# speechLabBcCuny/onssen

Measured on AMD Instinct MI355X. Metric: real_time_factor, higher is better.
Workload: dtype f32 as split-bf16 (bf16x3 MFMA, fp32 accumulate)

## Files before the change

### onssen_amd/_abi.py

```python
import ctypes as C
import os

EPI_BIAS, EPI_L2NORM, EPI_SIGMOID, EPI_RELU = 0, 1, 2, 3
EPI_BF16 = 0x100
ABI_VERSION = 14
WAV_TRUNCATED = 1
BLSTM_SPLIT_ROWS = 1
BLSTM_BF16X3 = 2
BLSTM_XCD = 4
BLSTM_FUSE_IN0 = 16
BLSTM_FUSE_TAIL = 32
BLSTM_BF16 = 64
BLSTM_G_READY = 128
BLSTM_WS_DIRTY = 65536
LSTM_BWD_STEPS, LSTM_BWD_XCD = 0, 1
DC_CLUSTER_LAUNCH_PER_ITERATION = 1
BLSTM_WS_HEADER = 32768
TASNET_GLN, TASNET_CLN, TASNET_BN = 0, 1, 2
TASNET_RELU, TASNET_SIGMOID, TASNET_SOFTMAX = 0, 1, 2
TASNET_RAGGED_MAX = 64
TASNET_F32, TASNET_BF16X3, TASNET_BF16 = 0, 1, 2

_vp, _i, _i64, _f, _sz = C.c_void_p, C.c_int, C.c_int64, C.c_float, C.c_size_t
_pp = C.POINTER(C.c_void_p)
# ... 508 lines not shown
    def cos_difference(self, s1, s2, n, out, stream):
        self.check(self.dll.onssen_cos_difference_f32(s1, s2, n, out, stream), "onssen_cos_difference_f32")

    def one_hot(self, feat, m1, m2, B, per_utt, db, utt_max, out, stream):
        self.check(self.dll.onssen_one_hot_f32(feat, m1, m2, B, per_utt, db, utt_max, out, stream), "onssen_one_hot_f32")

    def dc_compact_layout(self, B, T, F, D):
        co, do = _sz(), _sz()
        self.check(self.dll.onssen_dc_compact_layout(B, T, F, D, C.byref(co), C.byref(do)), "onssen_dc_compact_layout")
        return int(self.dll.onssen_dc_compact_workspace_bytes(B, T, F, D)), co.value, do.value

    def dc_index(self, feat, B, T, F, D, db, ws, ws_bytes, stream, frames=None):
        self.check(self.dll.onssen_dc_index_f32(feat, B, T, frames, F, D, db, ws, ws_bytes, stream), "onssen_dc_index_f32")

    def linear_x3p_compact(self, a_img, M, K, w_img, bias, N, group, eps, dest, dest_bs, F, comp, R, comp_bs, bf16_only, stream):
        self.check(self.dll.onssen_linear_x3p_compact(a_img, M, K, w_img, bias, N, group, eps, dest, dest_bs, F, comp, R, comp_bs,
                                                      int(bool(bf16_only)), stream), "onssen_linear_x3p_compact")

    def dc_cluster_compact(self, B, T, F, D, iters, masks, ws, ws_bytes, stream, flags=0, tol=1e-4):
        self.check(self.dll.onssen_dc_cluster_compact_f32(B, T, F, D, iters, tol, masks, ws, ws_bytes, flags, stream),
                   "onssen_dc_cluster_compact_f32")

    def dc_cluster(self, emb, feat, B, T, F, D, db, iters, masks, ws, ws_bytes, stream, flags=0, frames=None, tol=1e-4):
        if frames is not None:
            self.check(self.dll.onssen_dc_cluster_ragged_f32(emb, feat, B, T, frames, F, D, db, iters, tol, masks, ws, ws_bytes, flags,
                                                             stream), "onssen_dc_cluster_ragged_f32")
            return
        self.check(self.dll.onssen_dc_cluster_f32(emb, feat, B, T, F, D, db, iters, tol, masks, ws, ws_bytes, flags, stream),
                   "onssen_dc_cluster_f32")
```

### onssen_amd/csrc/gemm.inc

```
namespace lin {
constexpr int BM = 128, BN = 80, BK = 16;
constexpr int LD = 20;
constexpr int CLD = 84;
constexpr int STAGE = 2 * (BM + BN) * LD;
constexpr int SMEM = (BM * CLD > STAGE) ? BM * CLD : STAGE;
}

struct LinearArgs {
  const float* A;
  long a_s0, a_s1;
  const float* W;
  const float* bias;
  const float* resid;
  float* C;
  long c_s0, c_s1;
  int R, M, N, K, ldw, group;
  float eps;
};

__device__ __forceinline__ float f4c(const float4& v, int r) {
  return r == 0 ? v.x : (r == 1 ? v.y : (r == 2 ? v.z : v.w));
}

template <bool A_VEC, int MODE>
// ... 431 lines not shown
  long c_s0, c_s1;
  int R, M, N, KB, group;
  float eps;
  int tile_group;
  int c_vec;
  long a_bs, w_bs, c_bs;
  float* C2;
  long c2_s0, c2_s1, c2_bs;
  int n_split;
  int n_split_odd;
  const float* resid;
  int r_mod;
  const int* dest;
  long dest_bs;
  int F;
};

#ifndef ONSSEN_XP_ABLATE
#define ONSSEN_XP_ABLATE 0
#endif

template <int MODE, int WMS, int TERMS, bool BATCH = false>
__global__ __launch_bounds__(128 * WMS) void linear_x3p_kernel(LinearXpArgs p) {
  using namespace lxp;
  if constexpr (BATCH) {
    p.A += (long)blockIdx.z * p.a_bs;
    p.W += (long)blockIdx.z * p.w_bs;
    p.C += (long)blockIdx.z * p.c_bs;
    if (p.C2) p.C2 += (long)blockIdx.z * p.c2_bs;
    if (p.C2 && p.n_split_odd && (blockIdx.z & 1)) {
// ... 435 lines not shown
#define ONSSEN_XQ_STAGGER 0
#endif
#ifndef ONSSEN_XQ_WIDE_STORE
#define ONSSEN_XQ_WIDE_STORE 0
#endif
#ifndef ONSSEN_XQ_PRIO
#define ONSSEN_XQ_PRIO 0
#endif
#ifndef ONSSEN_XQ_STAGGER_PHASES
#define ONSSEN_XQ_STAGGER_PHASES 8
#endif
#define ONSSEN_EPI_L2NORM_SIGMOID 3
#define ONSSEN_EPI_L2NORM_COMPACT 4
namespace lxq {
constexpr int BM_MAX = 256;
}

template <int MODE, int TERMS, bool BATCH = false, int BN = 320, int BM = 256>
__global__ __launch_bounds__(512) void linear_x3q_kernel(LinearXpArgs p) {
  using namespace lxq;
  constexpr int STAGE = (BM + BN) * 128;
  constexpr int WN = BN / 4, NQW = (BM + BN) / 64;
  if constexpr (BATCH) {
    p.A += (long)blockIdx.z * p.a_bs;
    p.W += (long)blockIdx.z * p.w_bs;
    p.C += (long)blockIdx.z * p.c_bs;
  }
  constexpr int MT = BM / 32, NT = WN / 16, WM = BM / 2;
  __shared__ __attribute__((aligned(1024))) unsigned char stage0[STAGE];
  __shared__ __attribute__((aligned(1024))) unsigned char stage1[STAGE];
  const int tid = threadIdx.x, lane = tid & 63;
  const int wave = __builtin_amdgcn_readfirstlane(tid >> 6);
  const int wm = wave >> 2, wn = wave & 3;
  const int fi = lane & 15, fg = lane >> 4;
#if ONSSEN_XQ_STAGGER
  if (p.KB >= 16) {
    const int bl = blockIdx.y * gridDim.x + blockIdx.x;
    if (bl < 256) {
      const int ph = (bl >> 3) & (ONSSEN_XQ_STAGGER_PHASES - 1);
      for (int i = 0; i < ph; ++i) __builtin_amdgcn_s_sleep(ONSSEN_XQ_STAGGER);
    }
  }
#endif
  int n0, m0;
  {
    const int nbx = gridDim.x, nwg = nbx * gridDim.y, bid = blockIdx.y * nbx + blockIdx.x;
    const int q = nwg >> 3, r = nwg & 7, xcd = bid & 7;
    const int wg = (xcd < r ? xcd * (q + 1) : r * (q + 1) + (xcd - r) * q) + (bid >> 3);
    const int GN = p.tile_group, nby = gridDim.y;
    const int gfull = nbx / GN, nfull = gfull * GN * nby;
    int tn, tm;
    if (wg < nfull) {
      const int rem = wg % (nby * GN);
      tn = (wg / (nby * GN)) * GN + rem % GN;
      tm = rem / GN;
    } else {
      const int gl = nbx - gfull * GN, rem = wg - nfull;
      tn = gfull * GN + rem % gl;
      tm = rem / gl;
    }
    n0 = tn * BN;
    m0 = tm * BM;
  }
  const int pitch = p.KB * 128;
  const int a_rows = p.M - m0 < BM ? p.M - m0 : BM, w_rows = p.N - n0 < BN ? p.N - n0 : BN;
  const __amdgpu_buffer_rsrc_t ra = __builtin_amdgcn_make_buffer_rsrc(
      (void*)(p.A + (long)m0 * p.KB * 64), 0, a_rows * pitch, 0x00020000);
  const __amdgpu_buffer_rsrc_t rw = __builtin_amdgcn_make_buffer_rsrc(
      (void*)(p.W + (long)n0 * p.KB * 64), 0, w_rows * pitch, 0x00020000);
  const unsigned dma_lane = (unsigned)((lane >> 3) * pitch + (((lane & 7) ^ (lane >> 3)) * 16));
  auto dma = [&](unsigned char* stage, int kb) {
    const unsigned koff = (unsigned)(kb * 128);
#pragma unroll
    for (int j = 0; j < NQW; ++j) {
      const int q = wave * NQW + j;
      if (q < BM / 8)
        __builtin_amdgcn_raw_ptr_buffer_load_lds(ra, ONSSEN_LDS_PTR(stage + q * 1024), 16, dma_lane + (unsigned)(q * 8 * pitch) + koff, 0, 0, 0);
      else
        __builtin_amdgcn_raw_ptr_buffer_load_lds(rw, ONSSEN_LDS_PTR(stage + q * 1024), 16, dma_lane + (unsigned)((q - BM / 8) * 8 * pitch) + koff, 0, 0, 0);
    }
  };

  f32x4 acc[MT][NT];
#pragma unroll
  for (int mt = 0; mt < MT; ++mt)
#pragma unroll
    for (int nt = 0; nt < NT; ++nt) acc[mt][nt] = f32x4{0.f, 0.f, 0.f, 0.f};

  const unsigned ch = (unsigned)((fg ^ (fi & 7)) * 16), cl = ch ^ 64u;
  const unsigned fa_off = (unsigned)((wm * WM + fi) * 128);
  const unsigned fw_off = (unsigned)((BM + wn * WN + fi) * 128);
  auto compute = [&](const unsigned char* sb) {
    s16x8 wh[NT], wl[NT];
#pragma unroll
    for (int nt = 0; nt < NT; ++nt) {
// ... 40 lines not shown
      __builtin_amdgcn_s_waitcnt(0x0F70);
      __syncthreads();
    }
  }

  float4 bv[NT];
#pragma unroll
  for (int nt = 0; nt < NT; ++nt) {
    const int n = n0 + wn * WN + nt * 16 + 4 * fg;
    bv[nt].x = n + 0 < p.N ? p.bias[n + 0] : 0.f;
    bv[nt].y = n + 1 < p.N ? p.bias[n + 1] : 0.f;
    bv[nt].z = n + 2 < p.N ? p.bias[n + 2] : 0.f;
    bv[nt].w = n + 3 < p.N ? p.bias[n + 3] : 0.f;
  }
  u32x4 posv[MODE == ONSSEN_EPI_L2NORM_COMPACT ? MT : 1];
  if constexpr (MODE == ONSSEN_EPI_L2NORM_COMPACT) {
    const __amdgpu_buffer_rsrc_t rd = __builtin_amdgcn_make_buffer_rsrc((void*)p.dest, 0, (int)((long)p.R * p.dest_bs * 4 + 12), 0x00020000);
    const int f0 = (n0 + wn * WN) / p.group;
#pragma unroll
    for (int mt = 0; mt < MT; ++mt) {
      const int m = m0 + wm * WM + mt * 16 + fi;
      posv[mt] = __builtin_amdgcn_raw_buffer_load_b128(
          rd, m < p.M ? (unsigned)(((long)(m % p.R) * p.dest_bs + (long)(m / p.R) * p.F + f0) * 4) : 0x7ffffff0u, 0, 0);
    }
  }
#pragma unroll
  for (int mt = 0; mt < MT; ++mt) {
    const int m = m0 + wm * WM + mt * 16 + fi;
    float4 v[NT];
#pragma unroll
    for (int nt = 0; nt < NT; ++nt)
      v[nt] = make_float4(acc[mt][nt][0] + bv[nt].x, acc[mt][nt][1] + bv[nt].y, acc[mt][nt][2] + bv[nt].z,
                          acc[mt][nt][3] + bv[nt].w);
    if (MODE == ONSSEN_EPI_L2NORM && p.resid && m < p.M) {
      const float* rrow = p.resid + (long)(m / p.R) * p.c_s0 + (long)((m % p.R) % p.r_mod) * p.c_s1;
#pragma unroll
      for (int nt = 0; nt < NT; ++nt) {
        const int n = n0 + wn * WN + nt * 16 + 4 * fg;
// ... 38 lines not shown
        if (MODE == ONSSEN_EPI_L2NORM_SIGMOID && n0 + wn * WN + nt * 16 + 4 * fg >= p.n_split) {
          v[nt].x = 1.0f / (1.0f + expf(-v[nt].x)); v[nt].y = 1.0f / (1.0f + expf(-v[nt].y));
          v[nt].z = 1.0f / (1.0f + expf(-v[nt].z)); v[nt].w = 1.0f / (1.0f + expf(-v[nt].w));
        } else {
          v[nt].x *= sc; v[nt].y *= sc; v[nt].z *= sc; v[nt].w *= sc;
        }
      }
    } else if (MODE == ONSSEN_EPI_SIGMOID) {
#pragma unroll
      for (int nt = 0; nt < NT; ++nt) {
        v[nt].x = 1.0f / (1.0f + expf(-v[nt].x)); v[nt].y = 1.0f / (1.0f + expf(-v[nt].y));
        v[nt].z = 1.0f / (1.0f + expf(-v[nt].z)); v[nt].w = 1.0f / (1.0f + expf(-v[nt].w));
      }
    }
    if constexpr (MODE == ONSSEN_EPI_L2NORM_COMPACT) {
      if (m < p.M) {
        float* cb = p.C + (long)(m % p.R) * p.c_s1;
#pragma unroll
        for (int nt = 0; nt < NT; ++nt) {
          const int n = n0 + wn * WN + nt * 16 + 4 * fg, q = (nt * 16 + 4 * fg) / p.group;
          const int pos = (int)(q == 0 ? posv[mt][0] : q == 1 ? posv[mt][1] : q == 2 ? posv[mt][2] : posv[mt][3]);
          if (n < p.N && pos >= 0) *reinterpret_cast<float4*>(cb + (long)pos * p.group + (nt * 16 + 4 * fg) % p.group) = v[nt];
        }
      }
      continue;
    }
#if ONSSEN_XQ_WIDE_STORE
    if (MODE != ONSSEN_EPI_L2NORM_SIGMOID && p.c_vec) {
      const int mb = m0 + wm * WM + mt * 16, r8 = fi & 7;
      const int ma = mb + r8, mc = mb + r8 + 8;
      float* rowa = p.C + (long)(ma / p.R) * p.c_s0 + (long)(ma % p.R) * p.c_s1;
      float* rowc = p.C + (long)(mc / p.R) * p.c_s0 + (long)(mc % p.R) * p.c_s1;
// ... 292 lines not shown
```

### onssen_amd/csrc/labels_cluster.inc

```
__global__ void utt_max_kernel(const float* __restrict__ x, long per_utt, float* __restrict__ out) {
  __shared__ float red[256];
  const float* p = x + (long)blockIdx.x * per_utt;
  float m = -INFINITY;
  for (long i = threadIdx.x; i < per_utt; i += 256) m = fmaxf(m, p[i]);
  red[threadIdx.x] = m;
  __syncthreads();
  for (int s = 128; s > 0; s >>= 1) {
    if ((int)threadIdx.x < s) red[threadIdx.x] = fmaxf(red[threadIdx.x], red[threadIdx.x + s]);
    __syncthreads();
  }
  if (threadIdx.x == 0) out[blockIdx.x] = red[0];
}

__global__ void labels_kernel(const float* __restrict__ mix, const float* __restrict__ s1, const float* __restrict__ s2,
                              const float* __restrict__ feat, const float* __restrict__ fmax, long per_utt, long total,
                              float db_threshold, float* __restrict__ one_hot, float* __restrict__ mag_mix,
                              float* __restrict__ mag_s1, float* __restrict__ mag_s2, float* __restrict__ cos_s1,
                              float* __restrict__ cos_s2) {
  for (long e = (long)blockIdx.x * blockDim.x + threadIdx.x; e < total; e += (long)gridDim.x * blockDim.x) {
    const float xr = mix[2 * e], xi = mix[2 * e + 1];
    const float ar = s1[2 * e], ai = s1[2 * e + 1], br = s2[2 * e], bi = s2[2 * e + 1];
    const float m1 = hypotf(ar, ai), m2 = hypotf(br, bi);
    mag_mix[e] = hypotf(xr, xi);
    mag_s1[e] = m1;
// ... 727 lines not shown
  };
  if (fast) run(std::true_type{}); else run(std::false_type{});
  if (gave_up) return;
  if (j == 0) {
    if (tid < 2 * D) w[1 + tid] = cen[tid];
    if (tid == 0) {
      if (converged) w[ws_stride - 1] = 1.0f;
      iu[66] = it_done | (converged ? 0x10000 : 0) | (fast ? 0 : 0x20000);
    }
  }
}


__global__ __launch_bounds__(256) void kmeans2_index_kernel(const float* __restrict__ feat, long per_utt, float db,
                                                            const float* __restrict__ ws, long ws_stride, int* __restrict__ iw,
                                                            int* __restrict__ dest, const int* __restrict__ frames, int F, int D) {
  using namespace km;
  __shared__ int scan[256];
  __shared__ int base_s;
  const int b = blockIdx.y, tid = threadIdx.x;
  const float* f = feat + (long)b * per_utt;
  int* dst = dest + (long)b * per_utt;
  const float thr = ws[(long)b * ws_stride] - db / 20.0f;
  const long nb = frames ? (long)frames[b] * F : per_utt;
  const long chunk = (nb + NBLK - 1) / NBLK, i_lo = (long)blockIdx.x * chunk, i_hi = i_lo + chunk < nb ? i_lo + chunk : nb;
  if (tid == 0) {
    int sacc = 0;
    for (int k = 0; k < (int)blockIdx.x; ++k) sacc += iw[(long)b * IW + k];
    base_s = sacc;
    if (blockIdx.x == NBLK - 1) iw[(long)b * IW + 64] = sacc + iw[(long)b * IW + NBLK - 1];
  }
// ... 4 lines not shown
    const int act = (i < i_hi && f[i] >= thr) ? 1 : 0;
    scan[tid] = act;
    __syncthreads();
    for (int off = 1; off < 256; off <<= 1) {
      const int v = tid >= off ? scan[tid - off] : 0;
      __syncthreads();
      scan[tid] += v;
      __syncthreads();
    }
    if (i < i_hi) dst[i] = act ? base + scan[tid] - act : -1;
    const int tot = scan[255];
    __syncthreads();
    base += tot;
  }
  for (long i = nb + (long)blockIdx.x * 256 + tid; i < per_utt; i += (long)NBLK * 256) dst[i] = -1;
  if (blockIdx.x == 0) {
    float* wb = const_cast<float*>(ws) + (long)b * ws_stride;
    for (int k = tid; k < 2 * NBP * (D + 4); k += 256) wb[1 + 2 * D + k] = __builtin_bit_cast(float, 1u);
  }
}

template <int DT>
__global__ __launch_bounds__(256) void kmeans2_mask_compact_kernel(const float* __restrict__ comp, const int* __restrict__ dest,
                                                                   long per_utt, int D_rt, const float* __restrict__ ws,
                                                                   long ws_stride, float* __restrict__ masks) {
  using namespace km;
  constexpr int DC = DT ? DT : DMAX;
  const int D = DT ? DT : D_rt;
  const int b = blockIdx.y, tid = threadIdx.x;
  const float* e = comp + (long)b * per_utt * D;
  const int* dst = dest + (long)b * per_utt;
  const float* w = ws + (long)b * ws_stride;
  float c0[DC], c1[DC];
// ... 35 lines not shown
```

### onssen_amd/csrc/onssen_hip.hip

```cpp
#include <hip/hip_runtime.h>
#include <hip/hip_bf16.h>

#include <math.h>
#include <stdint.h>
#include <stdlib.h>

#include <type_traits>

#include "../../include/onssen_hip.h"

typedef float f32x4 __attribute__((vector_size(16)));
typedef unsigned int u32x4 __attribute__((vector_size(16)));
typedef unsigned int u32x2 __attribute__((vector_size(8)));
typedef short s16x8 __attribute__((vector_size(16)));
typedef __bf16 bf16x8_t __attribute__((vector_size(16)));

#ifdef ONSSEN_HOST_EMULATION
#define ONSSEN_USE_AFTER(x, after) ((void)0)
#define ONSSEN_LDS_PTR(p) ((void*)(p))
#else
#define ONSSEN_USE_AFTER(x, after) asm volatile("" : "+v"(x) : "v"(after))
#define ONSSEN_LDS_PTR(p) ((__attribute__((address_space(3))) void*)(p))
#endif

// ... 21 lines not shown
#define ONSSEN_LAUNCH_CHECK()                   \
  do {                                          \
    hipError_t e__ = hipGetLastError();         \
    if (e__ != hipSuccess) return (int)e__;     \
  } while (0)

static inline int ceil_div(int a, int b) { return (a + b - 1) / b; }
static inline size_t align256(size_t x) { return (x + 255) & ~(size_t)255; }
#ifdef ONSSEN_DEBUG_KNOBS
#define ONSSEN_KNOB_INT(name, dflt) (getenv(name) ? atoi(getenv(name)) : (dflt))
#else
#define ONSSEN_KNOB_INT(name, dflt) (dflt)
#endif
static inline bool aligned16(const void* p) { return (reinterpret_cast<uintptr_t>(p) & 15u) == 0; }
static inline bool aligned256(const void* p) { return (reinterpret_cast<uintptr_t>(p) & 255u) == 0; }
#ifndef ONSSEN_X3Q_SMALL_DEFAULT
#define ONSSEN_X3Q_SMALL_DEFAULT 0
#endif
#ifndef ONSSEN_X3R_DEFAULT
#define ONSSEN_X3R_DEFAULT 0
#endif

#include "pack.inc"
#include "gemm.inc"
#include "labels_cluster.inc"
#include "lstm.inc"
#include "lstm_bwd.inc"
#include "fft.inc"
#include "loss_sdr.inc"
#include "wav_io.inc"
// ... 351 lines not shown
                                   float* C2, int64_t c2_bs, int64_t c2_s0, int64_t c2_s1, int batch, void* stream,
                                   int n_split_odd = 0) {
  if (!a_img || !w_img || !bias || !C || M <= 0 || K <= 0 || N <= 0 || R <= 0 || batch <= 0 || batch > 65535) return ONSSEN_E_ARG;
  if (C2 && (n_split <= 0 || n_split >= N)) return ONSSEN_E_ARG;
  if (n_split_odd && (!C2 || n_split_odd < 0 || n_split_odd >= N)) return ONSSEN_E_ARG;
  if (!aligned16(a_img) || !aligned16(w_img) || (a_bs % 8) != 0 || (w_bs % 8) != 0) return ONSSEN_E_ALIGN;
  const int KB = ceil_div(K, 32);
  if ((long)lxp::BM * KB * 128 > 0x7fffffffL) return ONSSEN_E_ARG;
  ONSSEN_CLEAR_ERROR();
  LinearXpArgs p;
  p.A = a_img; p.W = w_img; p.bias = bias; p.C = C; p.c_s0 = (long)c_s0; p.c_s1 = (long)c_s1; p.R = R; p.M = M; p.N = N;
  p.KB = KB; p.group = 0; p.eps = 0.f; p.tile_group = 4;
  p.c_vec = !C2 && aligned16(C) && (N % 4) == 0 && (c_s0 % 4) == 0 && (c_s1 % 4) == 0 && (c_bs % 4) == 0;
  p.a_bs = (long)a_bs; p.w_bs = (long)w_bs; p.c_bs = (long)c_bs;
  p.C2 = C2; p.c2_s0 = (long)c2_s0; p.c2_s1 = (long)c2_s1; p.c2_bs = (long)c2_bs; p.n_split = n_split; p.n_split_odd = n_split_odd;
  p.resid = nullptr; p.r_mod = 1; p.dest = nullptr; p.dest_bs = 0; p.F = 0;
  const dim3 grid((unsigned)ceil_div(N, lxp::BN), (unsigned)ceil_div(M, lxp::BM), (unsigned)batch);
  hipLaunchKernelGGL((linear_x3p_kernel<ONSSEN_EPI_BIAS, 4, 3, true>), grid, dim3(512), 0, (hipStream_t)stream, p);
  ONSSEN_LAUNCH_CHECK();
  return ONSSEN_OK;
}

int onssen_linear_x3p_batched(const uint16_t* a_img, int64_t a_bs, int M, int K, const uint16_t* w_img, int64_t w_bs,
                              const float* bias, int N, float* C, int64_t c_bs, int64_t ldc, int batch, void* stream) {
  if (ldc < N) return ONSSEN_E_ARG;
  return linear_x3p_batched_impl(a_img, a_bs, M, K, w_img, w_bs, bias, N, 1, C, c_bs, ldc, 0, 0, nullptr, 0, 0, 0, batch, stream);
}

int onssen_linear_x3p_batched_split(const uint16_t* a_img, int64_t a_bs, int M, int K, const uint16_t* w_img, int64_t w_bs,
                                    const float* bias, int N, int R, float* C, int64_t c_bs, int64_t c_s0, int64_t c_s1,
                                    int n_split, float* C2, int64_t c2_bs, int64_t c2_s0, int64_t c2_s1, int batch, void* stream) {
// ... 71 lines not shown
  const bool bf16_only = (mode & ONSSEN_EPI_BF16) != 0;
  mode &= ~ONSSEN_EPI_BF16;
  const bool pairs = mode == ONSSEN_EPI_L2NORM && group == 2;
  if (mode == ONSSEN_EPI_L2NORM) {
    if (!pairs && (group <= 0 || (group % 4) != 0 || (80 % group) != 0 || 80 / group > 4)) return ONSSEN_E_ARG;
    if ((N % group) != 0) return ONSSEN_E_ARG;
  } else if (mode != ONSSEN_EPI_BIAS && mode != ONSSEN_EPI_SIGMOID) {
    return ONSSEN_E_ARG;
  }
  if (resid && (mode != ONSSEN_EPI_L2NORM || resid_mod <= 0)) return ONSSEN_E_ARG;
  if (inv_norm && (mode != ONSSEN_EPI_L2NORM || pairs)) return ONSSEN_E_ARG;
  ONSSEN_CLEAR_ERROR();
  LinearXpArgs p;
  p.A = a_img; p.W = w_img; p.bias = bias; p.C = C; p.c_s0 = (long)c_s0; p.c_s1 = (long)c_s1; p.R = R; p.M = M; p.N = N;
  p.KB = KB; p.group = group; p.eps = eps; p.resid = resid; p.r_mod = resid ? resid_mod : 1;
  p.dest = nullptr; p.dest_bs = 0; p.F = 0;
  p.a_bs = p.w_bs = p.c_bs = 0;
  p.C2 = inv_norm; p.c2_s0 = p.c2_s1 = p.c2_bs = 0; p.n_split = 0; p.n_split_odd = 0;
  static const int x3_gn = ONSSEN_KNOB_INT("ONSSEN_X3_GN", 4);
  p.tile_group = x3_gn < 1 ? 1 : x3_gn;
  p.c_vec = aligned16(C) && (N % 4) == 0 && (c_s0 % 4) == 0 && (c_s1 % 4) == 0;
  hipStream_t st = (hipStream_t)stream;
  const char* env_q = getenv("ONSSEN_X3Q");
  const char* env_bm = getenv("ONSSEN_X3Q_BM");
  const int use_q = (pairs || resid || inv_norm) ? 1 : env_q ? atoi(env_q) : 1, force_bm = env_bm ? atoi(env_bm) : 0;
  if ((pairs || resid || inv_norm) && (long)lxq::BM_MAX * KB * 128 > 0x7fffffffL) return ONSSEN_E_ARG;
  if (use_q && (long)lxq::BM_MAX * KB * 128 <= 0x7fffffffL) {
    int bm = 256, bn = 320;
    double best = 1e30;
    for (int cbm = 256; cbm >= 128; cbm -= 128)
      for (int cbn = 320; cbn >= 256; cbn -= 64) {
// ... 81 lines not shown
}

int onssen_linear_x3p_pair(const uint16_t* a_img, int M, int K, const uint16_t* w_img, const float* bias, int N, int n_split,
                           int group, float eps, float* C, int R, int64_t c_s0, int64_t c_s1, float* C2, int64_t c2_s0,
                           int64_t c2_s1, int bf16_only, void* stream) {
  if (!a_img || !w_img || !bias || !C || !C2 || R <= 0 || M <= 0 || K <= 0 || N <= 0) return ONSSEN_E_ARG;
  if (group <= 0 || (group % 4) != 0 || (80 % group) != 0 || 80 / group > 4) return ONSSEN_E_ARG;
  if (n_split <= 0 || n_split >= N || (n_split % group) != 0) return ONSSEN_E_ARG;
  if (!aligned16(a_img) || !aligned16(w_img)) return ONSSEN_E_ALIGN;
  const int KB = ceil_div(K, 32);
  if ((long)lxq::BM_MAX * KB * 128 > 0x7fffffffL) return ONSSEN_E_ARG;
  ONSSEN_CLEAR_ERROR();
  LinearXpArgs p;
  p.A = a_img; p.W = w_img; p.bias = bias; p.C = C; p.c_s0 = (long)c_s0; p.c_s1 = (long)c_s1; p.R = R; p.M = M; p.N = N;
  p.KB = KB; p.group = group; p.eps = eps; p.resid = nullptr; p.r_mod = 1;
  p.dest = nullptr; p.dest_bs = 0; p.F = 0;
  p.a_bs = p.w_bs = p.c_bs = 0;
  p.C2 = C2; p.c2_s0 = (long)c2_s0; p.c2_s1 = (long)c2_s1; p.c2_bs = 0; p.n_split = n_split; p.n_split_odd = 0;
  p.tile_group = 4;
  p.c_vec = aligned16(C) && (n_split % 4) == 0 && (c_s0 % 4) == 0 && (c_s1 % 4) == 0;
  const long t256 = (long)ceil_div(M, 256) * ceil_div(N, 320), t128 = (long)ceil_div(M, 128) * ceil_div(N, 320);
  const int bm = (double)ceil_div(t128, 256L) * 128 * 1.15 < (double)ceil_div(t256, 256L) * 256 ? 128 : 256;
  const dim3 gridq((unsigned)ceil_div(N, 320), (unsigned)ceil_div(M, bm));
  hipStream_t st = (hipStream_t)stream;
  if (bm == 256) { if (bf16_only) hipLaunchKernelGGL((linear_x3q_kernel<ONSSEN_EPI_L2NORM_SIGMOID, 1, false, 320, 256>), gridq, dim3(512), 0, st, p);
                   else hipLaunchKernelGGL((linear_x3q_kernel<ONSSEN_EPI_L2NORM_SIGMOID, 3, false, 320, 256>), gridq, dim3(512), 0, st, p); }
  else { if (bf16_only) hipLaunchKernelGGL((linear_x3q_kernel<ONSSEN_EPI_L2NORM_SIGMOID, 1, false, 320, 128>), gridq, dim3(512), 0, st, p);
         else hipLaunchKernelGGL((linear_x3q_kernel<ONSSEN_EPI_L2NORM_SIGMOID, 3, false, 320, 128>), gridq, dim3(512), 0, st, p); }
  ONSSEN_LAUNCH_CHECK();
  return ONSSEN_OK;
}
// ... 3 lines not shown
                              int bf16_only, void* stream) {
  if (!a_img || !w_img || !bias || !dest || !comp || R <= 0 || M <= 0 || K <= 0 || N <= 0 || F <= 0) return ONSSEN_E_ARG;
  if (group <= 0 || (group % 4) != 0 || (80 % group) != 0 || 80 / group > 4 || N != F * group) return ONSSEN_E_ARG;
  if (!aligned16(a_img) || !aligned16(w_img) || !aligned16(comp) || (comp_bs % 4) != 0) return ONSSEN_E_ALIGN;
  const int KB = ceil_div(K, 32);
  if ((long)lxq::BM_MAX * KB * 128 > 0x7fffffffL) return ONSSEN_E_ARG;
  ONSSEN_CLEAR_ERROR();
  LinearXpArgs p;
  p.A = a_img; p.W = w_img; p.bias = bias; p.C = comp; p.c_s0 = 0; p.c_s1 = (long)comp_bs; p.R = R; p.M = M; p.N = N;
  p.KB = KB; p.group = group; p.eps = eps; p.resid = nullptr; p.r_mod = 1;
  p.a_bs = p.w_bs = p.c_bs = 0;
  p.C2 = nullptr; p.c2_s0 = p.c2_s1 = p.c2_bs = 0; p.n_split = 0; p.n_split_odd = 0;
  p.dest = dest; p.dest_bs = (long)dest_bs; p.F = F;
  p.tile_group = 4;
  p.c_vec = 1;
  const long t256 = (long)ceil_div(M, 256) * ceil_div(N, 320), t128 = (long)ceil_div(M, 128) * ceil_div(N, 320);
  const int bm = (double)ceil_div(t128, 256L) * 128 * 1.15 < (double)ceil_div(t256, 256L) * 256 ? 128 : 256;
  const dim3 gridq((unsigned)ceil_div(N, 320), (unsigned)ceil_div(M, bm));
  hipStream_t st = (hipStream_t)stream;
  if (bm == 256) { if (bf16_only) hipLaunchKernelGGL((linear_x3q_kernel<ONSSEN_EPI_L2NORM_COMPACT, 1, false, 320, 256>), gridq, dim3(512), 0, st, p);
                   else hipLaunchKernelGGL((linear_x3q_kernel<ONSSEN_EPI_L2NORM_COMPACT, 3, false, 320, 256>), gridq, dim3(512), 0, st, p); }
  else { if (bf16_only) hipLaunchKernelGGL((linear_x3q_kernel<ONSSEN_EPI_L2NORM_COMPACT, 1, false, 320, 128>), gridq, dim3(512), 0, st, p);
         else hipLaunchKernelGGL((linear_x3q_kernel<ONSSEN_EPI_L2NORM_COMPACT, 3, false, 320, 128>), gridq, dim3(512), 0, st, p); }
  ONSSEN_LAUNCH_CHECK();
  return ONSSEN_OK;
}

int onssen_linear_x3p_resid(const uint16_t* a_img, int M, int K, const uint16_t* w_img, const float* bias, int N, int group,
                            float eps, const float* resid, int resid_mod, float* C, int R, int64_t c_s0, int64_t c_s1,
                            int bf16_only, void* stream) {
  if (group != 2 && (group <= 0 || (group % 4) != 0)) return ONSSEN_E_ARG;
  return linear_x3p_impl(a_img, M, K, w_img, bias, N, ONSSEN_EPI_L2NORM | (bf16_only ? ONSSEN_EPI_BF16 : 0), group, eps, resid,
// ... 950 lines not shown
    }
  } else {
    hipLaunchKernelGGL((kmeans2_search_kernel<1>), sgrid, dim3(256), 0, st, emb, feature, per_utt, D, db_threshold, w, stride, frames, F);
    hipLaunchKernelGGL((kmeans2_pick_kernel<1>), dim3((unsigned)B), dim3(64), 0, st, emb, per_utt, D, w, stride, (int*)nullptr);
    for (int it = 0; it < iters; ++it) {
      ONSSEN_KM_ASSIGN(0, (float*)nullptr);
      hipLaunchKernelGGL(kmeans2_update_kernel, dim3((unsigned)B), dim3(256), 0, st, D, km::NBLK, w, stride, tol);
    }
  }
  ONSSEN_KM_ASSIGN(1, masks);
#undef ONSSEN_KM_ASSIGN
  ONSSEN_LAUNCH_CHECK();
  return ONSSEN_OK;
}

size_t onssen_dc_compact_workspace_bytes(int B, int T, int F, int D) {
  const size_t base = onssen_dc_cluster_workspace_bytes(B, T, F, D);
  return base ? align256(base) + align256((size_t)B * T * F * sizeof(int32_t) + 16) : 0;
}

int onssen_dc_compact_layout(int B, int T, int F, int D, size_t* comp_offset, size_t* dest_offset) {
  if (onssen_dc_cluster_workspace_bytes(B, T, F, D) == 0) return ONSSEN_E_ARG;
  if (comp_offset) *comp_offset = align256(onssen_dc_cluster_status_offset(B, D) + 256);
  if (dest_offset) *dest_offset = align256(onssen_dc_cluster_workspace_bytes(B, T, F, D));
  return ONSSEN_OK;
}

int onssen_dc_index_f32(const float* feature, int B, int T, const int32_t* frames, int F, int D, float db_threshold, void* ws,
                        size_t ws_bytes, void* stream) {
  if (!feature || !ws || B <= 0 || T <= 0 || F <= 0 || D <= 0 || D > km::DMAX) return ONSSEN_E_ARG;
  if (ws_bytes < onssen_dc_compact_workspace_bytes(B, T, F, D)) return ONSSEN_E_WORKSPACE;
  if (reinterpret_cast<uintptr_t>(ws) & 255u) return ONSSEN_E_ALIGN;
  ONSSEN_CLEAR_ERROR();
  hipStream_t st = (hipStream_t)stream;
  const long per_utt = (long)T * F, stride = 1 + 2 * D + km::NBLK * 2 * (D + 1) + 1;
  float* w = (float*)ws;
  int* iw = (int*)((char*)ws + align256(dc_cluster_header_floats(B, D) * sizeof(float)));
  size_t dest_off = 0;
  onssen_dc_compact_layout(B, T, F, D, nullptr, &dest_off);
  int* dest = (int*)((char*)ws + dest_off);
  const dim3 sgrid(km::NBLK, (unsigned)B);
  hipLaunchKernelGGL((kmeans2_search_kernel<0>), sgrid, dim3(256), 0, st, (const float*)nullptr, feature, per_utt, D, db_threshold, w, stride, frames, F);
  hipLaunchKernelGGL((kmeans2_count_kernel<true>), sgrid, dim3(256), 0, st, feature, per_utt, db_threshold, w, stride, iw, frames, F, D);
  hipLaunchKernelGGL(kmeans2_index_kernel, sgrid, dim3(256), 0, st, feature, per_utt, db_threshold, (const float*)w, stride, iw, dest, frames, F, D);
  ONSSEN_LAUNCH_CHECK();
  return ONSSEN_OK;
}

int onssen_dc_cluster_compact_f32(int B, int T, int F, int D, int iters, float tol, float* masks, void* ws, size_t ws_bytes,
                                  int flags, void* stream) {
  if (!masks || !ws || B <= 0 || T <= 0 || F <= 0 || D <= 0 || D > km::DMAX || iters < 0 || !(tol >= 0.f)) return ONSSEN_E_ARG;
  if (flags & ONSSEN_DC_CLUSTER_LAUNCH_PER_ITERATION) return ONSSEN_E_ARG;
  if (ws_bytes < onssen_dc_compact_workspace_bytes(B, T, F, D)) return ONSSEN_E_WORKSPACE;
  if (reinterpret_cast<uintptr_t>(ws) & 255u) return ONSSEN_E_ALIGN;
  ONSSEN_CLEAR_ERROR();
  hipStream_t st = (hipStream_t)stream;
  const long per_utt = (long)T * F, stride = 1 + 2 * D + km::NBLK * 2 * (D + 1) + 1;
  float* w = (float*)ws;
  int* iw = (int*)((char*)ws + align256(dc_cluster_header_floats(B, D) * sizeof(float)));
// ... 104 lines not shown
```

### onssen_amd/options.py

```python
import os

_BOOL = {True: "1", False: "0", "1": "1", "0": "0", "true": "1", "false": "0", "on": "1", "off": "0"}


def _choice(*allowed):
    def conv(v):
        v = str(v).lower() if not isinstance(v, bool) else _BOOL[v]
        if v not in allowed:
            raise ValueError(f"must be one of {allowed}, got {v!r}")
        return v
    return conv


def _flag(v):
    try:
        return _BOOL[v if isinstance(v, bool) else str(v).lower()]
    except KeyError:
        raise ValueError(f"must be a boolean, got {v!r}") from None


def _alias(table):
    def conv(v):
        k = _BOOL.get(v, None) if isinstance(v, bool) else str(v).lower()
        if k in table:
# ... 23 lines not shown
    "split_rows": ("ONSSEN_SPLIT_ROWS", "0", _flag, "launch-per-step recurrence: split the batch rows over two workgroups"),
    "ablate": ("ONSSEN_ABLATE", "0", _int, "profiling-only ablation bits of the recurrence kernels"),
    "serialize_persistent": ("ONSSEN_XCD_SERIALIZE", "0", _flag, "one persistent launch in flight per device across streams"),
    "nonfinite": ("ONSSEN_NONFINITE", "propagate", _choice("raise", "propagate"),
                  "non-finite activations seen by a persistent launch (they cannot pass its tagged exchange): propagate (default since round 6) = the "
                  "call is re-run on the launch-per-step recurrence, which gives nn.LSTM's NaN in / NaN out -- the reference's behaviour --; "
                  "raise = stop with an error instead"),
    "check": ("ONSSEN_CHECK", "0", _flag, "synchronise and examine the persistent launches' status words after every forward"),
    "check_weights": ("ONSSEN_CHECK_WEIGHTS", "0", _flag, "verify the packed weight images against the parameters before every forward (one synchronisation each: debugging)"),
    "weight_guard": ("ONSSEN_WEIGHT_GUARD", "1", _flag, "every inference forward that reuses cached weight images compares a device-side sampled checksum of the "
                     "live parameters with the one taken when the images were built (one small launch, no synchronisation); a mismatch drops the "
                     "images and raises StalePackedWeights at the next status poll (separate_* / tester.eval re-run the call by themselves)"),
    "dc_cluster": ("ONSSEN_DC_PERSISTENT", "1", _alias({"persistent": "1", "steps": "0"}),
                   "deep-clustering 2-means: all Lloyd passes in one launch, or one launch per pass"),
    "dc_compact": ("ONSSEN_DC_COMPACT", "1", _flag, "fc_dc stores only the active bins' embeddings into the clustering's array"),
    "train_blstm": ("ONSSEN_TRAIN_HIP", "1", _alias({"hip": "1", "aten": "0"}), "training BLSTM / head / BatchNorm on the HIP kernels"),
    "train_backward": ("ONSSEN_BWD_XCD", "1", _alias({"persistent": "1", "steps": "0"}), "backward recurrence form"),
    "train_gemm": ("ONSSEN_TRAIN_GEMM", "x3", _choice("x3", "blas"), "weight / input gradient contractions: package GEMM or library fp32"),
    "train_dp_image": ("ONSSEN_TRAIN_DP_IMAGE", "1", _flag, "the backward recurrence writes dP as the gradient GEMMs' x3 image instead of fp32"),
    "train_wgrad_rows": ("ONSSEN_TRAIN_WGRAD_ROWS", "1", _flag, "weight gradients from the row-major images the forward left"),
    "train_fused_loss": ("ONSSEN_TRAIN_FUSED_LOSS", "1", _flag, "fc_dc + normalise + loss_dc as one autograd node in train_step"),
    "train_fused_norm": ("ONSSEN_TRAIN_FUSED_NORM", "1", _flag, "fc_dc + normalise as one autograd node"),
    "tasnet_train": ("ONSSEN_TASNET_TRAIN", "hip", _choice("hip", "aten"),
                     "ConvTasNet training: hip = forward and backward of the network on the HIP kernels behind one autograd node "
                     "(gln / cln; bn, an input that requires a gradient and anomaly mode go to ATen by themselves), aten = autograd over PyTorch ops"),
    "loss": ("ONSSEN_LOSS_HIP", "1", _alias({"hip": "1", "torch": "0"}), "loss kernels on the device or PyTorch ops"),
    "fused_adam": ("ONSSEN_FUSED_ADAM", "1", _flag, "build_optimizer returns utils.ClipAdam (clipping + Adam on onssen_clip_adam_f32) for device parameters"),
    "cpu_autograd": ("ONSSEN_CPU_AUTOGRAD", "0", _flag, "TEST SCAFFOLDING, off in the product: let a training forward on CPU tensors run on ATen's LSTM so that "
                     "the multi-process logic (gradient buckets, replica agreement) can be exercised over gloo without a GPU; otherwise a CPU tensor raises"),
    "synthetic_data": ("ONSSEN_SYNTHETIC_DATA", "0", _flag, "wsj0_2mix_dataloader falls back to the synthetic corpus when data_path is empty"),
# ... 3 lines not shown
}

_configured = {}


def get(key):
    env, default, _, _ = TABLE[key]
    v = os.environ.get(env)
    if v is not None:
        return v
    return _configured.get(key, default)


def flag(key):
    return get(key) == "1"


def configure(**kw):
    old = {}
    for k, v in kw.items():
        if k not in TABLE:
            raise KeyError(f"onssen_amd.options: unknown option {k!r} (known: {sorted(TABLE)})")
        old[k] = _configured.get(k)
        if v is None:
            _configured.pop(k, None)
            continue
        try:
            _configured[k] = TABLE[k][2](v)
        except ValueError as e:
            raise ValueError(f"onssen_amd.options: {k} {e}") from None
# ... 36 lines not shown
```

Before: 67090.

## Add per-column-tile row lists so compacted fc_dc GEMM skips inactive rows

The index kernel now also writes per-row flags saying whether each 320-column tile has an active bin, and a new kernel scans them into per-tile row lists. The compact L2-norm GEMM can then gather only the listed rows through buffer-load offsets, and it exits early for tiles past the list length. The path is gated by ONSSEN_DC_ROWS, which defaults to 0, so by default only the extra flag writes and the row-list kernel run. That adds work to the indexing step and grows the workspace.

```diff
diff --git a/onssen_amd/_abi.py b/onssen_amd/_abi.py
--- a/onssen_amd/_abi.py
+++ b/onssen_amd/_abi.py
@@ -546,6 +546,8 @@
         self.check(self.dll.onssen_dc_index_f32(feat, B, T, frames, F, D, db, ws, ws_bytes, stream), "onssen_dc_index_f32")
 
     def linear_x3p_compact(self, a_img, M, K, w_img, bias, N, group, eps, dest, dest_bs, F, comp, R, comp_bs, bf16_only, stream):
+        from . import options
+        options.export_native("dc_rows")
         self.check(self.dll.onssen_linear_x3p_compact(a_img, M, K, w_img, bias, N, group, eps, dest, dest_bs, F, comp, R, comp_bs,
                                                       int(bool(bf16_only)), stream), "onssen_linear_x3p_compact")
 
diff --git a/onssen_amd/csrc/gemm.inc b/onssen_amd/csrc/gemm.inc
--- a/onssen_amd/csrc/gemm.inc
+++ b/onssen_amd/csrc/gemm.inc
@@ -469,6 +469,7 @@
   const int* dest;
   long dest_bs;
   int F;
+  const int* rows;
 };
 
 #ifndef ONSSEN_XP_ABLATE
@@ -934,6 +935,22 @@
 #define ONSSEN_EPI_L2NORM_COMPACT 4
 namespace lxq {
 constexpr int BM_MAX = 256;
+constexpr int ROWS_MAGIC = 0x52574c53, ROWS_HDR = 8, ROWS_BN = 320;
+__host__ __device__ inline int rows_hdr_ints(int ncols) { return ((ROWS_HDR + ncols) * 4 + 255) / 256 * 64; }
+}
+
+template <int BM, int NQW, bool ROWS>
+__device__ __forceinline__ void x3q_dma(__amdgpu_buffer_rsrc_t ra, __amdgpu_buffer_rsrc_t rw, unsigned char* stage, int kb, int wave,
+                                        unsigned dma_lane, int pitch, const unsigned* a_off) {
+  const unsigned koff = (unsigned)(kb * 128);
+#pragma unroll
+  for (int j = 0; j < NQW; ++j) {
+    const int q = wave * NQW + j;
+    if (q < BM / 8)
+      __builtin_amdgcn_raw_ptr_buffer_load_lds(ra, ONSSEN_LDS_PTR(stage + q * 1024), 16, (ROWS ? a_off[ROWS ? j : 0] : dma_lane + (unsigned)(q * 8 * pitch)) + koff, 0, 0, 0);
+    else
+      __builtin_amdgcn_raw_ptr_buffer_load_lds(rw, ONSSEN_LDS_PTR(stage + q * 1024), 16, dma_lane + (unsigned)((q - BM / 8) * 8 * pitch) + koff, 0, 0, 0);
+  }
 }
 
 template <int MODE, int TERMS, bool BATCH = false, int BN = 320, int BM = 256>
@@ -953,6 +970,7 @@
   const int wave = __builtin_amdgcn_readfirstlane(tid >> 6);
   const int wm = wave >> 2, wn = wave & 3;
   const int fi = lane & 15, fg = lane >> 4;
+  constexpr bool ROWS = MODE == ONSSEN_EPI_L2NORM_COMPACT;
 #if ONSSEN_XQ_STAGGER
   if (p.KB >= 16) {
     const int bl = blockIdx.y * gridDim.x + blockIdx.x;
@@ -963,6 +981,7 @@
   }
 #endif
   int n0, m0;
+  const int* rlist = nullptr;
   {
     const int nbx = gridDim.x, nwg = nbx * gridDim.y, bid = blockIdx.y * nbx + blockIdx.x;
     const int q = nwg >> 3, r = nwg & 7, xcd = bid & 7;
@@ -981,24 +1000,34 @@
     }
     n0 = tn * BN;
     m0 = tm * BM;
+    if constexpr (ROWS) {
+      if (p.rows && p.rows[0] == ROWS_MAGIC && p.rows[1] == p.M && p.rows[2] == nbx && p.rows[4] == p.group && p.rows[5] == p.F) {
+        if (m0 >= p.rows[ROWS_HDR + tn]) return;
+        rlist = p.rows + rows_hdr_ints(nbx) + (long)tn * p.rows[3] + m0;
+      }
+    }
   }
   const int pitch = p.KB * 128;
   const int a_rows = p.M - m0 < BM ? p.M - m0 : BM, w_rows = p.N - n0 < BN ? p.N - n0 : BN;
   const __amdgpu_buffer_rsrc_t ra = __builtin_amdgcn_make_buffer_rsrc(
-      (void*)(p.A + (long)m0 * p.KB * 64), 0, a_rows * pitch, 0x00020000);
+      (void*)(p.A + (ROWS && rlist ? 0L : (long)m0 * p.KB * 64)), 0, (ROWS && rlist ? p.M : a_rows) * pitch, 0x00020000);
   const __amdgpu_buffer_rsrc_t rw = __builtin_amdgcn_make_buffer_rsrc(
       (void*)(p.W + (long)n0 * p.KB * 64), 0, w_rows * pitch, 0x00020000);
   const unsigned dma_lane = (unsigned)((lane >> 3) * pitch + (((lane & 7) ^ (lane >> 3)) * 16));
-  auto dma = [&](unsigned char* stage, int kb) {
-    const unsigned koff = (unsigned)(kb * 128);
+  unsigned a_off[ROWS ? NQW : 1] = {0u};
+  if constexpr (ROWS) {
 #pragma unroll
     for (int j = 0; j < NQW; ++j) {
       const int q = wave * NQW + j;
-      if (q < BM / 8)
-        __builtin_amdgcn_raw_ptr_buffer_load_lds(ra, ONSSEN_LDS_PTR(stage + q * 1024), 16, dma_lane + (unsigned)(q * 8 * pitch) + koff, 0, 0, 0);
-      else
-        __builtin_amdgcn_raw_ptr_buffer_load_lds(rw, ONSSEN_LDS_PTR(stage + q * 1024), 16, dma_lane + (unsigned)((q - BM / 8) * 8 * pitch) + koff, 0, 0, 0);
-    }
+      a_off[j] = dma_lane + (unsigned)(q * 8 * pitch);
+      if (rlist && q < BM / 8) {
+        const int r = rlist[q * 8 + (lane >> 3)];
+        a_off[j] = r >= 0 ? (unsigned)(r * pitch + (((lane & 7) ^ (lane >> 3)) * 16)) : 0x80000000u;
+      }
+    }
+  }
+  auto dma = [&](unsigned char* stage, int kb) {
+    x3q_dma<BM, NQW, ROWS>(ra, rw, stage, kb, wave, dma_lane, pitch, a_off);
   };
 
   f32x4 acc[MT][NT];
@@ -1069,14 +1098,20 @@
     bv[nt].w = n + 3 < p.N ? p.bias[n + 3] : 0.f;
   }
   u32x4 posv[MODE == ONSSEN_EPI_L2NORM_COMPACT ? MT : 1];
+  int mrow[ROWS ? MT : 1];
   if constexpr (MODE == ONSSEN_EPI_L2NORM_COMPACT) {
     const __amdgpu_buffer_rsrc_t rd = __builtin_amdgcn_make_buffer_rsrc((void*)p.dest, 0, (int)((long)p.R * p.dest_bs * 4 + 12), 0x00020000);
     const int f0 = (n0 + wn * WN) / p.group;
 #pragma unroll
     for (int mt = 0; mt < MT; ++mt) {
-      const int m = m0 + wm * WM + mt * 16 + fi;
+      const int md = m0 + wm * WM + mt * 16 + fi;
+      mrow[mt] = rlist ? rlist[wm * WM + mt * 16 + fi] : md < p.M ? md : -1;
+    }
+#pragma unroll
+    for (int mt = 0; mt < MT; ++mt) {
+      const int m = mrow[mt];
       posv[mt] = __builtin_amdgcn_raw_buffer_load_b128(
-          rd, m < p.M ? (unsigned)(((long)(m % p.R) * p.dest_bs + (long)(m / p.R) * p.F + f0) * 4) : 0x7ffffff0u, 0, 0);
+          rd, m >= 0 ? (unsigned)(((long)(m % p.R) * p.dest_bs + (long)(m / p.R) * p.F + f0) * 4) : 0x7ffffff0u, 0, 0);
     }
   }
 #pragma unroll
@@ -1145,8 +1180,8 @@
       }
     }
     if constexpr (MODE == ONSSEN_EPI_L2NORM_COMPACT) {
-      if (m < p.M) {
-        float* cb = p.C + (long)(m % p.R) * p.c_s1;
+      if (mrow[mt] >= 0) {
+        float* cb = p.C + (long)(mrow[mt] % p.R) * p.c_s1;
 #pragma unroll
         for (int nt = 0; nt < NT; ++nt) {
           const int n = n0 + wn * WN + nt * 16 + 4 * fg, q = (nt * 16 + 4 * fg) / p.group;
diff --git a/onssen_amd/csrc/labels_cluster.inc b/onssen_amd/csrc/labels_cluster.inc
--- a/onssen_amd/csrc/labels_cluster.inc
+++ b/onssen_amd/csrc/labels_cluster.inc
@@ -765,7 +765,8 @@
 
 __global__ __launch_bounds__(256) void kmeans2_index_kernel(const float* __restrict__ feat, long per_utt, float db,
                                                             const float* __restrict__ ws, long ws_stride, int* __restrict__ iw,
-                                                            int* __restrict__ dest, const int* __restrict__ frames, int F, int D) {
+                                                            int* __restrict__ dest, const int* __restrict__ frames, int F, int D,
+                                                            unsigned char* __restrict__ rflags, long rf_stride, int ncols) {
   using namespace km;
   __shared__ int scan[256];
   __shared__ int base_s;
@@ -800,9 +801,63 @@
     base += tot;
   }
   for (long i = nb + (long)blockIdx.x * 256 + tid; i < per_utt; i += (long)NBLK * 256) dst[i] = -1;
+  if (rflags) {
+    const int bpc = lxq::ROWS_BN / D, nseg = (int)(per_utt / F) * ncols, per = (nseg + NBLK - 1) / NBLK;
+    const int s_hi = ((int)blockIdx.x + 1) * per < nseg ? ((int)blockIdx.x + 1) * per : nseg;
+    for (int sg = (int)blockIdx.x * per + tid; sg < s_hi; sg += 256) {
+      const int t = sg / ncols, c = sg - t * ncols;
+      const int f_lo = c * bpc, f_hi = f_lo + bpc < F ? f_lo + bpc : F;
+      int any = 0;
+      if ((long)t * F < nb)
+        for (int k = f_lo; k < f_hi; ++k) any |= f[(long)t * F + k] >= thr ? 1 : 0;
+      rflags[(long)c * rf_stride + (long)t * gridDim.y + b] = (unsigned char)any;
+    }
+  }
   if (blockIdx.x == 0) {
     float* wb = const_cast<float*>(ws) + (long)b * ws_stride;
     for (int k = tid; k < 2 * NBP * (D + 4); k += 256) wb[1 + 2 * D + k] = __builtin_bit_cast(float, 1u);
+  }
+}
+
+__global__ __launch_bounds__(256) void kmeans2_rows_kernel(const unsigned char* __restrict__ rflags, long rf_stride, int M, int ncols,
+                                                           int ls, int D, int F, int* __restrict__ hdr, int* __restrict__ rows) {
+  __shared__ int scan[256];
+  const int s = blockIdx.x, c = blockIdx.y, tid = threadIdx.x;
+  const unsigned* fw = reinterpret_cast<const unsigned*>(rflags + (long)c * rf_stride);
+  int* out = rows + (long)c * ls;
+  int cnt = 0;
+  for (int w = tid; w < s * 256; w += 256) cnt += __builtin_popcount(fw[w] & 0x01010101u);
+  scan[tid] = cnt;
+  __syncthreads();
+  for (int s2 = 128; s2 > 0; s2 >>= 1) {
+    if (tid < s2) scan[tid] += scan[tid + s2];
+    __syncthreads();
+  }
+  const int base = scan[0];
+  __syncthreads();
+  const int m4 = (s * 256 + tid) * 4;
+  unsigned word = m4 < M ? fw[s * 256 + tid] & 0x01010101u : 0u;
+  if (m4 + 4 > M) word &= m4 < M ? (0x01010101u >> (8 * (m4 + 4 - M))) : 0u;
+  const int n = __builtin_popcount(word);
+  scan[tid] = n;
+  __syncthreads();
+  for (int off = 1; off < 256; off <<= 1) {
+    const int v = tid >= off ? scan[tid - off] : 0;
+    __syncthreads();
+    scan[tid] += v;
+    __syncthreads();
+  }
+  int pos = base + scan[tid] - n;
+#pragma unroll
+  for (int k = 0; k < 4; ++k)
+    if ((word >> (8 * k)) & 1u) out[pos++] = m4 + k;
+  if (s == (int)gridDim.x - 1) {
+    const int total = base + scan[255];
+    for (int i = total + tid; i < (total + 255) / 256 * 256; i += 256) out[i] = -1;
+    if (tid == 0) {
+      hdr[lxq::ROWS_HDR + c] = total;
+      if (c == 0) { hdr[1] = M; hdr[2] = ncols; hdr[3] = ls; hdr[4] = D; hdr[5] = F; hdr[0] = lxq::ROWS_MAGIC; }
+    }
   }
 }
 
diff --git a/onssen_amd/csrc/onssen_hip.hip b/onssen_amd/csrc/onssen_hip.hip
--- a/onssen_amd/csrc/onssen_hip.hip
+++ b/onssen_amd/csrc/onssen_hip.hip
@@ -59,6 +59,9 @@
 #endif
 static inline bool aligned16(const void* p) { return (reinterpret_cast<uintptr_t>(p) & 15u) == 0; }
 static inline bool aligned256(const void* p) { return (reinterpret_cast<uintptr_t>(p) & 255u) == 0; }
+#ifndef ONSSEN_DC_ROWS_DEFAULT
+#define ONSSEN_DC_ROWS_DEFAULT 0
+#endif
 #ifndef ONSSEN_X3Q_SMALL_DEFAULT
 #define ONSSEN_X3Q_SMALL_DEFAULT 0
 #endif
@@ -440,7 +443,7 @@
   p.c_vec = !C2 && aligned16(C) && (N % 4) == 0 && (c_s0 % 4) == 0 && (c_s1 % 4) == 0 && (c_bs % 4) == 0;
   p.a_bs = (long)a_bs; p.w_bs = (long)w_bs; p.c_bs = (long)c_bs;
   p.C2 = C2; p.c2_s0 = (long)c2_s0; p.c2_s1 = (long)c2_s1; p.c2_bs = (long)c2_bs; p.n_split = n_split; p.n_split_odd = n_split_odd;
-  p.resid = nullptr; p.r_mod = 1; p.dest = nullptr; p.dest_bs = 0; p.F = 0;
+  p.resid = nullptr; p.r_mod = 1; p.dest = nullptr; p.dest_bs = 0; p.F = 0; p.rows = nullptr;
   const dim3 grid((unsigned)ceil_div(N, lxp::BN), (unsigned)ceil_div(M, lxp::BM), (unsigned)batch);
   hipLaunchKernelGGL((linear_x3p_kernel<ONSSEN_EPI_BIAS, 4, 3, true>), grid, dim3(512), 0, (hipStream_t)stream, p);
   ONSSEN_LAUNCH_CHECK();
@@ -542,7 +545,7 @@
   LinearXpArgs p;
   p.A = a_img; p.W = w_img; p.bias = bias; p.C = C; p.c_s0 = (long)c_s0; p.c_s1 = (long)c_s1; p.R = R; p.M = M; p.N = N;
   p.KB = KB; p.group = group; p.eps = eps; p.resid = resid; p.r_mod = resid ? resid_mod : 1;
-  p.dest = nullptr; p.dest_bs = 0; p.F = 0;
+  p.dest = nullptr; p.dest_bs = 0; p.F = 0; p.rows = nullptr;
   p.a_bs = p.w_bs = p.c_bs = 0;
   p.C2 = inv_norm; p.c2_s0 = p.c2_s1 = p.c2_bs = 0; p.n_split = 0; p.n_split_odd = 0;
   static const int x3_gn = ONSSEN_KNOB_INT("ONSSEN_X3_GN", 4);
@@ -654,7 +657,7 @@
   LinearXpArgs p;
   p.A = a_img; p.W = w_img; p.bias = bias; p.C = C; p.c_s0 = (long)c_s0; p.c_s1 = (long)c_s1; p.R = R; p.M = M; p.N = N;
   p.KB = KB; p.group = group; p.eps = eps; p.resid = nullptr; p.r_mod = 1;
-  p.dest = nullptr; p.dest_bs = 0; p.F = 0;
+  p.dest = nullptr; p.dest_bs = 0; p.F = 0; p.rows = nullptr;
   p.a_bs = p.w_bs = p.c_bs = 0;
   p.C2 = C2; p.c2_s0 = (long)c2_s0; p.c2_s1 = (long)c2_s1; p.c2_bs = 0; p.n_split = n_split; p.n_split_odd = 0;
   p.tile_group = 4;
@@ -688,8 +691,14 @@
   p.dest = dest; p.dest_bs = (long)dest_bs; p.F = F;
   p.tile_group = 4;
   p.c_vec = 1;
+  const char* env_rows = getenv("ONSSEN_DC_ROWS");
+  const bool use_rows = (env_rows ? atoi(env_rows) != 0 : ONSSEN_DC_ROWS_DEFAULT != 0) && (long)M * KB * 128 < 0x7fffffffL;
+  p.rows = use_rows ? dest + align256((size_t)R * (size_t)dest_bs * sizeof(int32_t) + 16) / sizeof(int32_t) : nullptr;
   const long t256 = (long)ceil_div(M, 256) * ceil_div(N, 320), t128 = (long)ceil_div(M, 128) * ceil_div(N, 320);
-  const int bm = (double)ceil_div(t128, 256L) * 128 * 1.15 < (double)ceil_div(t256, 256L) * 256 ? 128 : 256;
+  const char* env_bm = getenv("ONSSEN_DC_ROWS_BM");
+  const int force_bm = env_bm ? atoi(env_bm) : 0;
+  const int bm = force_bm == 128 || force_bm == 256 ? force_bm
+                 : (double)ceil_div(t128, 256L) * 128 * 1.15 < (double)ceil_div(t256, 256L) * 256 ? 128 : 256;
   const dim3 gridq((unsigned)ceil_div(N, 320), (unsigned)ceil_div(M, bm));
   hipStream_t st = (hipStream_t)stream;
   if (bm == 256) { if (bf16_only) hipLaunchKernelGGL((linear_x3q_kernel<ONSSEN_EPI_L2NORM_COMPACT, 1, false, 320, 256>), gridq, dim3(512), 0, st, p);
@@ -1670,9 +1679,15 @@
   return ONSSEN_OK;
 }
 
+static inline int dc_rows_cols(int F, int D) { return ceil_div(F * D, lxq::ROWS_BN); }
+static inline long dc_rows_stride(int B, int T) { return ((long)B * T + 255) / 256 * 256; }
+static size_t dc_rows_bytes(int B, int T, int F, int D) {
+  const size_t nc = (size_t)dc_rows_cols(F, D), ls = (size_t)dc_rows_stride(B, T);
+  return (size_t)lxq::rows_hdr_ints((int)nc) * 4 + nc * ls * 4 + align256(nc * ls);
+}
 size_t onssen_dc_compact_workspace_bytes(int B, int T, int F, int D) {
   const size_t base = onssen_dc_cluster_workspace_bytes(B, T, F, D);
-  return base ? align256(base) + align256((size_t)B * T * F * sizeof(int32_t) + 16) : 0;
+  return base ? align256(base) + align256((size_t)B * T * F * sizeof(int32_t) + 16) + dc_rows_bytes(B, T, F, D) : 0;
 }
 
 int onssen_dc_compact_layout(int B, int T, int F, int D, size_t* comp_offset, size_t* dest_offset) {
@@ -1698,7 +1713,17 @@
   const dim3 sgrid(km::NBLK, (unsigned)B);
   hipLaunchKernelGGL((kmeans2_search_kernel<0>), sgrid, dim3(256), 0, st, (const float*)nullptr, feature, per_utt, D, db_threshold, w, stride, frames, F);
   hipLaunchKernelGGL((kmeans2_count_kernel<true>), sgrid, dim3(256), 0, st, feature, per_utt, db_threshold, w, stride, iw, frames, F, D);
-  hipLaunchKernelGGL(kmeans2_index_kernel, sgrid, dim3(256), 0, st, feature, per_utt, db_threshold, (const float*)w, stride, iw, dest, frames, F, D);
+  const bool lists = (lxq::ROWS_BN % D) == 0 && (long)B * T < 0x7fffff00L;
+  const int ncols = dc_rows_cols(F, D);
+  const long ls = dc_rows_stride(B, T);
+  int* hdr = (int*)((char*)dest + align256((size_t)B * T * F * sizeof(int32_t) + 16));
+  int* rows = hdr + lxq::rows_hdr_ints(ncols);
+  unsigned char* rflags = (unsigned char*)(rows + (size_t)ncols * ls);
+  hipLaunchKernelGGL(kmeans2_index_kernel, sgrid, dim3(256), 0, st, feature, per_utt, db_threshold, (const float*)w, stride, iw, dest, frames, F, D,
+                     lists ? rflags : (unsigned char*)nullptr, ls, ncols);
+  if (lists)
+    hipLaunchKernelGGL(kmeans2_rows_kernel, dim3((unsigned)ceil_div(B * T, 1024), (unsigned)ncols), dim3(256), 0, st,
+                       (const unsigned char*)rflags, ls, B * T, ncols, (int)ls, D, F, hdr, rows);
   ONSSEN_LAUNCH_CHECK();
   return ONSSEN_OK;
 }
diff --git a/onssen_amd/options.py b/onssen_amd/options.py
--- a/onssen_amd/options.py
+++ b/onssen_amd/options.py
@@ -61,6 +61,9 @@
     "dc_cluster": ("ONSSEN_DC_PERSISTENT", "1", _alias({"persistent": "1", "steps": "0"}),
                    "deep-clustering 2-means: all Lloyd passes in one launch, or one launch per pass"),
     "dc_compact": ("ONSSEN_DC_COMPACT", "1", _flag, "fc_dc stores only the active bins' embeddings into the clustering's array"),
+    "dc_rows": ("ONSSEN_DC_ROWS", "0", _flag, "compacted fc_dc GEMM: a 320-column tile multiplies only the rows that have an active bin among its "
+                "columns (row lists written with the target map); 0 = every row.  Same bits either way.  The native library reads the "
+                "environment variable per call: a configured value is exported by export_native() before the launch"),
     "train_blstm": ("ONSSEN_TRAIN_HIP", "1", _alias({"hip": "1", "aten": "0"}), "training BLSTM / head / BatchNorm on the HIP kernels"),
     "train_backward": ("ONSSEN_BWD_XCD", "1", _alias({"persistent": "1", "steps": "0"}), "backward recurrence form"),
     "train_gemm": ("ONSSEN_TRAIN_GEMM", "x3", _choice("x3", "blas"), "weight / input gradient contractions: package GEMM or library fp32"),
@@ -94,6 +97,12 @@
 
 def flag(key):
     return get(key) == "1"
+
+
+def export_native(key):
+    env = TABLE[key][0]
+    if key in _configured and os.environ.get(env) is None:
+        os.environ[env] = _configured[key]
 
 
 def configure(**kw):
```

Measured after the change: 66150. -1.4%, worse.
